# buctcurry/ICKA

Measured on AMD Instinct MI355X. Metric: MNER samples/sec (fwd+bwd) at seq=128, 36 regions, bs=32 per GPU, higher is better.
Workload: dtype bf16; 1 GPU; c2: bert(H768,L12,h12,I3072)+36x2048 regions, seq_len 128, per-GPU batch 32, 1 cross layer(s), gated head, 13 labels, train mode p=0.1, token-CE loss; global_batch=32, seq_len=128, regions=36, parallelism=dp1, launch=hipgraph, precision=bf16, accumulate=1

## Files before the change

### icka_amd/_lib.py

```python
from __future__ import annotations

import ctypes as C
import os
from typing import Optional

_HERE = os.path.dirname(os.path.abspath(__file__))
LIB_PATH = os.path.join(_HERE, "libicka_hip.so")

c_vp, c_i32, c_i64, c_u64, c_f32 = C.c_void_p, C.c_int32, C.c_int64, C.c_uint64, C.c_float

ABI_VERSION = 6
GEMM_NT, GEMM_NN, GEMM_TN, GEMM_TT = 0, 1, 2, 3
ATTN_FP8, ATTN_TILED = 1, 2
LSTM_PER_STEP, LSTM_TICKETS, LSTM_NO_BATCH_SPLIT = 1, 2, 4
EPI_NONE, EPI_GELU, EPI_DGELU, EPI_ADD, EPI_GATE, EPI_TANH, EPI_RELU, EPI_ADD_RELU = 0, 1, 2, 3, 4, 5, 6, 7


class GemmDesc(C.Structure):
    _fields_ = [
        ("op", c_i32), ("M", c_i32), ("N", c_i32), ("K", c_i32), ("K1", c_i32),
        ("A", c_vp), ("lda", c_i64), ("B", c_vp), ("ldb", c_i64),
        ("A2", c_vp), ("lda2", c_i64), ("B2", c_vp), ("ldb2", c_i64),
        ("C", c_vp), ("ldc", c_i64), ("c_is_f32", c_i32),
        ("C2", c_vp), ("ldc2", c_i64),
        ("aux", c_vp), ("ldaux", c_i64),
        ("bias", c_vp), ("bias2", c_vp),
        ("alpha", c_f32), ("beta", c_f32),
        ("epilogue", c_i32),
# ... 228 lines not shown
```

### icka_amd/csrc/attention.hip

```cpp
#include "attn_core.h"

namespace {

__global__ __launch_bounds__(256) void attn_fwd_kernel(const AttnArgs a_) {
    AttnArgs a = a_;
    a.drop = drop_resolve(a.drop);
    __shared__ __attribute__((aligned(16))) char smem[3 * TILE_B];
    char* sQ = smem; char* sK = smem + TILE_B; char* sV = smem + 2 * TILE_B;
    const int tid = threadIdx.x, lane = tid & 63, wave = tid >> 6, g = lane >> 4, i15 = lane & 15;
    const int nqt = (a.Sq + TILE - 1) / TILE;
    const int qt = blockIdx.x % nqt, bh = blockIdx.x / nqt, head = bh % a.h, b = bh / a.h;
    const bf16_t* Qb = a.Q + (int64_t)b * a.Sq * a.ldq + head * HD;
    const bf16_t* Kb = a.K + (int64_t)b * a.Skv * a.ldk + head * HD;
    const bf16_t* Vb = a.V + (int64_t)b * a.Skv * a.ldv + head * HD;
    const float* mb = a.mask + (int64_t)b * a.Skv;

    stage_tile(sQ, Qb, a.ldq, qt * TILE, a.Sq, tid);
    __syncthreads();
    bf16x8 qf[2];
    qf[0] = frag_row(sQ, 16 * wave, 0, lane);
    qf[1] = frag_row(sQ, 16 * wave, 1, lane);
    const int q = qt * TILE + 16 * wave + i15;
    const uint32_t idx_row = ((uint32_t)(b * a.h + head) * (uint32_t)a.Sq + (uint32_t)q) * (uint32_t)a.Skv;

// ... 449 lines not shown
        return;
    }
    if (ICKA_ATTN_ABLATE == 2) {
        for (int i = 0; i < QR * 8 / 256; ++i) {
            const int q = tid + 256 * i, r = q >> 3, c = q & 7;
            if (q0 + r < a.Sq) *reinterpret_cast<u32x4*>(a.Ow + ((int64_t)b * a.Sq + q0 + r) * a.ldo + head * HD + c * 8) =
                *reinterpret_cast<const u32x4*>(sQ + off_t(r, c)) ^ *reinterpret_cast<const u32x4*>(sK + off_t(r % KR, c)) ^
                *reinterpret_cast<const u32x4*>(sV + off_t(r % KR, c));
        }
        return;
    }

    attn_fwd_whole_head<QT, KT, DROP, FP8, KB>(a, sQ, sK, sV, QT * wave, q0, bh, b, head, lane);
}

template <int QT, int KT, bool DROP, bool KB = false, bool VL = false>
__global__ __launch_bounds__(256, (QT * KT >= 36 || QT >= 4 ? 1 : 2)) void attn_bwd_small_kernel(const AttnArgs a_) {
    static_assert(DROP || !KB, "keep bits exist with dropout only");
    static_assert(!(VL && QT * KT >= 36), "packed batches: heads of up to 128 x 128");
    AttnArgs a = a_;
    a.drop = drop_resolve(a.drop);
    constexpr int QR = 64 * QT, KR = 16 * KT, KW = KT / 4;
    constexpr int KV_BYTES = 2 * KR * 128, CH_BYTES = QR * 128;
    constexpr int X_BYTES = KV_BYTES > CH_BYTES ? KV_BYTES : CH_BYTES;
    constexpr int NCAP = (X_BYTES / CH_BYTES) < KW ? (X_BYTES / CH_BYTES) : KW;
    constexpr int NCH = KW % NCAP == 0 ? NCAP : 1;
    constexpr int NG = KW / NCH;
    static_assert(KW % NCH == 0, "chunk groups");
    constexpr bool MASK_LDS = QT * KT >= 36;
    __shared__ __attribute__((aligned(16))) char smem[2 * QR * 128 + X_BYTES + QR * 4 + (MASK_LDS ? KR * 4 : 0)];
    char* sQ = smem; char* sDO = smem + QR * 128; char* sK = sDO + QR * 128; char* sV = sK + KR * 128;
    float* s_lse = reinterpret_cast<float*>(sK + X_BYTES);
    float* s_mask = s_lse + QR;
    const int tid = threadIdx.x, lane = tid & 63, wave = tid >> 6, g = lane >> 4, i15 = lane & 15;
    const int bh = blockIdx.x, head = bh % a.h, b = bh / a.h;
    const float* mb = a.mask + (int64_t)b * a.Skv;
    ATTN_RSTAMP(8);
    ATTN_STAMP(0);
    int qlim = a.Sq, kvlim = a.Skv;
    int64_t q_row0 = (int64_t)b * a.Sq, kv_row0 = (int64_t)b * a.Skv;
    if constexpr (VL) {
        if (bh >= a.B * a.h) {
            const int fb = bh - a.B * a.h;
            vl_zero_filler(a, a.dQ, a.lddq, fb, tid);
            if (a.kv_packed) {
// ... 8 lines not shown
            if (!a.kv_packed) {
                for (int i = tid; i < a.Skv * 8; i += 256) {
                    const int r = i >> 3, c = i & 7;
                    *reinterpret_cast<u32x4*>(a.dK + (kv_row0 + r) * a.lddk + head * HD + c * 8) = u32x4{0u, 0u, 0u, 0u};
                    *reinterpret_cast<u32x4*>(a.dV + (kv_row0 + r) * a.lddv + head * HD + c * 8) = u32x4{0u, 0u, 0u, 0u};
                }
            }
            return;
        }
    }
    stage_rows<QR>(sQ, a.Q + q_row0 * a.ldq + head * HD, a.ldq, qlim, tid);
    stage_rows<QR>(sDO, a.dO + q_row0 * a.lddo + head * HD, a.lddo, qlim, tid);
    stage_rows<KR>(sK, a.K + kv_row0 * a.ldk + head * HD, a.ldk, kvlim, tid);
    stage_rows<KR>(sV, a.V + kv_row0 * a.ldv + head * HD, a.ldv, kvlim, tid);
    if (tid < QR) s_lse[tid] = tid < qlim ? a.lse[(int64_t)bh * a.Sq + tid] : INFINITY;
    if constexpr (MASK_LDS) {
        static_assert(KR <= 256, "one mask element per thread");
        if (tid < KR) s_mask[tid] = tid < a.Skv ? mb[tid] : -INFINITY;
    }
    ATTN_STAMP(1);
    __syncthreads();
    ATTN_STAMP(2);
    if (ICKA_ATTN_ABLATE == 2 && !VL) {
        for (int i = 0; i < QR * 8 / 256; ++i) {
            const int q = tid + 256 * i, r = q >> 3, c = q & 7;
            if (r < a.Sq) *reinterpret_cast<u32x4*>(a.dQ + ((int64_t)b * a.Sq + r) * a.lddq + head * HD + c * 8) =
                *reinterpret_cast<const u32x4*>(sQ + off_t(r, c)) ^ *reinterpret_cast<const u32x4*>(sDO + off_t(r, c));
        }
        for (int i = 0; i < KR * 8 / 256; ++i) {
            const int q = tid + 256 * i, r = q >> 3, c = q & 7;
            if (r < a.Skv) {
                *reinterpret_cast<u32x4*>(a.dK + ((int64_t)b * a.Skv + r) * a.lddk + head * HD + c * 8) =
                    *reinterpret_cast<const u32x4*>(sK + off_t(r, c));
                *reinterpret_cast<u32x4*>(a.dV + ((int64_t)b * a.Skv + r) * a.lddv + head * HD + c * 8) =
                    *reinterpret_cast<const u32x4*>(sV + off_t(r, c));
            }
        }
        return;
    }

    f32x4 mk[MASK_LDS ? 1 : KT];
    if constexpr (!MASK_LDS) {
#pragma unroll
        for (int kt = 0; kt < KT; ++kt)
#pragma unroll
            for (int r = 0; r < 4; ++r) {
                const int key = 16 * kt + 4 * g + r;
                const float mv = mb[key < a.Skv ? key : a.Skv - 1];
                mk[kt][r] = key < a.Skv ? mv : -INFINITY;
            }
    }
    constexpr bool DROP_BITS = MASK_LDS && DROP;
    constexpr int KBW = (KT * 4 + 31) / 32;
    const int wpl = keep_wpl(a.Skv);
    uint32_t dbits[DROP_BITS ? (QT * KT * 4 + 31) / 32 : 1];
    if constexpr (DROP_BITS) {
#pragma unroll
        for (int w = 0; w < (QT * KT * 4 + 31) / 32; ++w) dbits[w] = 0u;
#pragma unroll
        for (int qi = 0; qi < QT; ++qi) {
            const int q = 16 * (QT * wave + qi) + i15;
            const uint32_t idx_row = ((uint32_t)bh * (uint32_t)a.Sq + (uint32_t)q) * (uint32_t)a.Skv;
            const uint32_t hx = (idx_row + 2u * (uint32_t)g) * ICKA_HASH_C0 + a.drop.s0;
            uint32_t kbw[KBW];
            if constexpr (KB) {
// ... 5 lines not shown
            for (int kt = 0; kt < KT; ++kt) {
                const int bit = (qi * KT + kt) * 4;
                uint32_t nib;
                if constexpr (KB) nib = (kbw[(kt * 4) >> 5] >> ((kt * 4) & 31)) & 0xFu;
                else nib = drop_nibble_x<true>(a.drop, hx + (uint32_t)(8 * kt) * ICKA_HASH_C0);
                dbits[bit >> 5] |= nib << (bit & 31);
            }
        }
#pragma unroll
        for (int w = 0; w < (QT * KT * 4 + 31) / 32; ++w) asm volatile("" : "+v"(dbits[w]));
    }
    u32x2 pdp[QT][KT], dsp[QT][KT];
#pragma unroll
    for (int qi = 0; qi < QT; ++qi) {
        const int q = 16 * (QT * wave + qi) + i15;
        if constexpr (VL) {
            if (16 * (QT * wave + qi) >= qlim) {
#pragma unroll
                for (int kt = 0; kt < KT; ++kt) pdp[qi][kt] = dsp[qi][kt] = u32x2{0u, 0u};
                continue;
            }
        }
        const bf16x8 qf0 = frag_row(sQ, 16 * (QT * wave + qi), 0, lane), qf1 = frag_row(sQ, 16 * (QT * wave + qi), 1, lane);
        const bf16x8 do0 = frag_row(sDO, 16 * (QT * wave + qi), 0, lane), do1 = frag_row(sDO, 16 * (QT * wave + qi), 1, lane);
        const float lse_q = s_lse[q];
        const uint32_t idx_row = ((uint32_t)bh * (uint32_t)a.Sq + (uint32_t)q) * (uint32_t)a.Skv;
        const uint32_t hx = (idx_row + 2u * (uint32_t)g) * ICKA_HASH_C0 + a.drop.s0;
        uint32_t kbw[KBW];
        if constexpr (KB && !DROP_BITS) {
            const uint32_t* kp = a.keepbits + (((int64_t)bh * a.Sq + (q < qlim ? q : 0)) * 4 + g) * wpl;
#pragma unroll
            for (int w = 0; w < KBW; ++w) kbw[w] = (w < wpl && q < qlim) ? kp[w] : 0u;
        }
        f32x4 pr[MASK_LDS ? 1 : KT], dpm[KT];
        float dl = 0.f;
#pragma unroll
        for (int kt = 0; kt < KT; ++kt) {
            f32x4 sc = mfma16(frag_row(sK, 16 * kt, 0, lane), qf0, f32x4{0.f, 0.f, 0.f, 0.f});
            sc = mfma16(frag_row(sK, 16 * kt, 1, lane), qf1, sc);
            f32x4 dp = mfma16(frag_row(sV, 16 * kt, 0, lane), do0, f32x4{0.f, 0.f, 0.f, 0.f});
            dp = mfma16(frag_row(sV, 16 * kt, 1, lane), do1, dp);
            f32x4 pd, pvv;
            f32x4 mkv;
            if constexpr (MASK_LDS) mkv = *reinterpret_cast<const f32x4*>(s_mask + 16 * kt + 4 * g);
            else mkv = mk[kt];
            const uint32_t hk = hx + (uint32_t)(8 * kt) * ICKA_HASH_C0;
            if constexpr (MASK_LDS) __builtin_amdgcn_sched_barrier(0);
            float dm4[4];
            if constexpr (!DROP_BITS) {
                if constexpr (KB) {
                    const uint32_t w = kbw[(kt * 4) >> 5], sb = __float_as_uint(a.drop.scale);
#pragma unroll
                    for (int r = 0; r < 4; ++r)
                        dm4[r] = __uint_as_float(sb & (uint32_t)__builtin_amdgcn_sbfe((int)w, ((kt * 4) & 31) + r, 1));
                } else {
                    drop_pair_x<DROP>(a.drop, hk, dm4[0], dm4[1]);
                    drop_pair_x<DROP>(a.drop, hk + ICKA_HASH_C0, dm4[2], dm4[3]);
                }
            }
#pragma unroll
            for (int r = 0; r < 4; ++r) {
                const float pv = __expf(sc[r] * a.scale + mkv[r] - lse_q);
                float dm;
                if constexpr (DROP_BITS) {
                    const int bit = (qi * KT + kt) * 4 + r;
                    dm = ((dbits[bit >> 5] >> (bit & 31)) & 1u) ? a.drop.scale : 0.f;
                } else {
                    dm = dm4[r];
                }
                const float dv = dp[r] * dm;
                pvv[r] = pv;
                dpm[kt][r] = dv;
                pd[r] = pv * dm;
                dl += pv * dv;
            }
            if constexpr (MASK_LDS) {
                pdp[qi][kt] = pack4(pvv[0], pvv[1], pvv[2], pvv[3]);
            } else {
                pr[kt] = pvv;
                pdp[qi][kt] = pack4(pd[0], pd[1], pd[2], pd[3]);
            }
        }
        dl += __shfl_xor(dl, 16, 64);
        dl += __shfl_xor(dl, 32, 64);
        if (g == 0 && q < qlim) a.delta[(int64_t)bh * a.Sq + q] = dl;
#pragma unroll
        for (int kt = 0; kt < KT; ++kt) {
            f32x4 pk;
            if constexpr (MASK_LDS) {
                const bf16x4 pb = as_bf16x4(pdp[qi][kt]);
                pk = f32x4{bf2f(pb[0]), bf2f(pb[1]), bf2f(pb[2]), bf2f(pb[3])};
            } else {
                pk = pr[kt];
            }
            const f32x4 d = pk * (dpm[kt] - dl) * a.scale;
            dsp[qi][kt] = pack4(d[0], d[1], d[2], d[3]);
        }
        f32x4 acc[4];
#pragma unroll
        for (int dt = 0; dt < 4; ++dt) {
            acc[dt] = f32x4{0.f, 0.f, 0.f, 0.f};
#pragma unroll
            for (int ks = 0; ks < KT / 2; ++ks)
                acc[dt] = mfma16(frag_tr(sK, dt, ks, lane),
                                 join8(as_bf16x4(dsp[qi][2 * ks]), as_bf16x4(dsp[qi][2 * ks + 1])), acc[dt]);
        }
        if (q < qlim) {
            bf16_t* row = a.dQ + (q_row0 + q) * a.lddq + head * HD;
#pragma unroll
            for (int dt = 0; dt < 4; ++dt)
                *reinterpret_cast<u32x2*>(row + 16 * dt + 4 * g) = pack4(acc[dt][0], acc[dt][1], acc[dt][2], acc[dt][3]);
        }
    }

    ATTN_STAMP(3);
    char* sX = sK;
    f32x4 acc_k[KW][4], acc_v[KW][4];
#pragma unroll
    for (int kw = 0; kw < KW; ++kw)
#pragma unroll
// ... 61 lines not shown
            if (key < kvlim) {
                bf16_t* krow = a.dK + (kv_row0 + key) * a.lddk + head * HD;
                bf16_t* vrow = a.dV + (kv_row0 + key) * a.lddv + head * HD;
#pragma unroll
                for (int dt = 0; dt < 4; ++dt) {
                    *reinterpret_cast<u32x2*>(krow + 16 * dt + 4 * g) =
                        pack4(acc_k[kw][dt][0], acc_k[kw][dt][1], acc_k[kw][dt][2], acc_k[kw][dt][3]);
                    *reinterpret_cast<u32x2*>(vrow + 16 * dt + 4 * g) =
                        pack4(acc_v[kw][dt][0], acc_v[kw][dt][1], acc_v[kw][dt][2], acc_v[kw][dt][3]);
                }
            }
        }
    ATTN_RSTAMP(9);
}

template <int QT, int KT, bool DROP, bool KB>
static void launch_small2(const AttnArgs& a, int mode, hipStream_t st) {
    if (mode == 1) {
        hipLaunchKernelGGL((attn_bwd_small_kernel<QT, KT, DROP, KB>), dim3(a.B * a.h), dim3(256), 0, st, a);
        return;
    }
    if constexpr (QT > 2) return;
    else if (QT == 2 && (a.B * a.h) % 256 != 0) {
        if (mode == 2) hipLaunchKernelGGL((attn_fwd_small_kernel<1, KT, DROP, true, KB>), dim3(a.B * a.h, 2), dim3(256), 0, st, a);
        else hipLaunchKernelGGL((attn_fwd_small_kernel<1, KT, DROP, false, KB>), dim3(a.B * a.h, 2), dim3(256), 0, st, a);
        return;
    }
    if constexpr (QT <= 2) {
        if (mode == 2) hipLaunchKernelGGL((attn_fwd_small_kernel<QT, KT, DROP, true, KB>), dim3(a.B * a.h), dim3(256), 0, st, a);
        else hipLaunchKernelGGL((attn_fwd_small_kernel<QT, KT, DROP, false, KB>), dim3(a.B * a.h), dim3(256), 0, st, a);
    }
}
template <int QT, int KT>
static void launch_small(const AttnArgs& a, int mode, hipStream_t st) {
    if (a.drop.thr && a.keepbits) launch_small2<QT, KT, true, true>(a, mode, st);
    else if (a.drop.thr) launch_small2<QT, KT, true, false>(a, mode, st);
    else launch_small2<QT, KT, false, false>(a, mode, st);
}
template <int KT>
static void launch_small_fwd_blocks(const AttnArgs& a, hipStream_t st) {
    const dim3 grid(a.B * a.h, (a.Sq + 63) / 64);
    if (a.drop.thr && a.keepbits) hipLaunchKernelGGL((attn_fwd_small_kernel<1, KT, true, false, true>), grid, dim3(256), 0, st, a);
    else if (a.drop.thr) hipLaunchKernelGGL((attn_fwd_small_kernel<1, KT, true, false, false>), grid, dim3(256), 0, st, a);
    else hipLaunchKernelGGL((attn_fwd_small_kernel<1, KT, false, false, false>), grid, dim3(256), 0, st, a);
}
static bool try_small(const AttnArgs& a, int mode, hipStream_t st) {
    if (mode == 0 && a.Skv <= 256 && (a.Sq > 128 || a.Skv > 128)) {
        if (a.Skv > 192) launch_small_fwd_blocks<16>(a, st);
        else if (a.Skv > 128) launch_small_fwd_blocks<12>(a, st);
        else if (a.Skv > 64) launch_small_fwd_blocks<8>(a, st);
        else launch_small_fwd_blocks<4>(a, st);
        return true;
    }
    if (mode == 1 && a.Sq <= 256 && a.Skv <= 256 && (a.Sq > 128 || a.Skv > 128)) {
        if (a.Sq <= 192 && a.Skv <= 192 && a.Skv > 128) launch_small<3, 12>(a, mode, st);
        else if (a.Skv > 128) launch_small<4, 16>(a, mode, st);
        else if (a.Skv > 64) launch_small<4, 8>(a, mode, st);
        else launch_small<4, 4>(a, mode, st);
        return true;
    }
    if (a.Sq > 128 || a.Skv > 128) return false;
    const bool q2 = a.Sq > 64, k8 = a.Skv > 64;
    if (q2 && k8) launch_small<2, 8>(a, mode, st);
    else if (q2) launch_small<2, 4>(a, mode, st);
    else if (k8) launch_small<1, 8>(a, mode, st);
    else launch_small<1, 4>(a, mode, st);
    return true;
}

template <int QT, int KT, bool DROP, bool KB>
static void launch_vl2(const AttnArgs& a, bool bwd, hipStream_t st) {
    const int nb = a.B * a.h + VL_FILL_BLOCKS;
    if (bwd) {
        hipLaunchKernelGGL((attn_bwd_small_kernel<QT, KT, DROP, KB, true>), dim3(nb), dim3(256), 0, st, a);
    } else if (QT == 2 && (a.B * a.h) % 256 != 0) {
        hipLaunchKernelGGL((attn_fwd_small_kernel<1, KT, DROP, false, KB, true>), dim3(nb, 2), dim3(256), 0, st, a);
    } else {
        hipLaunchKernelGGL((attn_fwd_small_kernel<QT, KT, DROP, false, KB, true>), dim3(nb), dim3(256), 0, st, a);
    }
}
template <int QT, int KT>
static void launch_vl(const AttnArgs& a, bool bwd, hipStream_t st) {
    if (a.drop.thr && a.keepbits) launch_vl2<QT, KT, true, true>(a, bwd, st);
    else if (a.drop.thr) launch_vl2<QT, KT, true, false>(a, bwd, st);
    else launch_vl2<QT, KT, false, false>(a, bwd, st);
}
static void try_vl(const AttnArgs& a, bool bwd, hipStream_t st) {
    const bool q2 = a.Sq > 64, k8 = a.Skv > 64;
    if (q2 && k8) launch_vl<2, 8>(a, bwd, st);
    else if (q2) launch_vl<2, 4>(a, bwd, st);
    else if (k8) launch_vl<1, 8>(a, bwd, st);
    else launch_vl<1, 4>(a, bwd, st);
}

inline bool ok16(const void* p, int64_t ld) { return (reinterpret_cast<uintptr_t>(p) & 15) == 0 && ld % 8 == 0; }

#ifdef ICKA_ATTN_STAMP
unsigned long long* g_attn_stamp = nullptr;
#endif

}

#ifdef ICKA_ATTN_STAMP
extern "C" void icka_diag_attn_stamp_buffer(void* p) { g_attn_stamp = (unsigned long long*)p; }
#endif

extern "C" int icka_attn_fwd(const void* Q, int64_t ldq, const void* K, int64_t ldk, const void* V, int64_t ldv,
                             const float* add_mask, void* O, int64_t ldo, float* lse, int32_t B, int32_t heads,
                             int32_t Sq, int32_t Skv, float scale, float p_drop, uint64_t seed, void* stream) {
    if (!Q || !K || !V || !add_mask || !O) return ICKA_E_ARG;
// ... 67 lines not shown
        ICKA_CHECK_LAUNCH();
    }
    return 0;
}
extern "C" int64_t icka_attn_keepbits_words(int32_t B, int32_t heads, int32_t Sq, int32_t Skv) {
    if (B <= 0 || heads <= 0 || Sq <= 0 || Skv <= 0) return 0;
    return (int64_t)B * heads * Sq * 4 * ((Skv + 127) >> 7);
}

extern "C" int icka_attn_bwd(const void* Q, int64_t ldq, const void* K, int64_t ldk, const void* V, int64_t ldv,
                             const float* add_mask, const void* O, int64_t ldo, const void* dO, int64_t lddo,
                             const float* lse, float* delta, void* dQ, int64_t lddq, void* dK, int64_t lddk,
                             void* dV, int64_t lddv, int32_t B, int32_t heads, int32_t Sq, int32_t Skv, float scale,
                             float p_drop, uint64_t seed, const void* keep_bits, int32_t flags, void* stream) {
    if (!Q || !K || !V || !add_mask || !O || !dO || !lse || !delta || !dQ || !dK || !dV) return ICKA_E_ARG;
    if (flags & ~ICKA_ATTN_TILED) return ICKA_E_ARG;
    if (B <= 0 || heads <= 0 || Sq <= 0 || Skv <= 0) return ICKA_E_SHAPE;
    if ((int64_t)B * heads * Sq * Skv >= (1ll << 32)) return ICKA_E_SHAPE;
    if (!ok16(Q, ldq) || !ok16(K, ldk) || !ok16(V, ldv) || !ok16(O, ldo) || !ok16(dO, lddo) || !ok16(dQ, lddq) ||
        !ok16(dK, lddk) || !ok16(dV, lddv))
        return ICKA_E_ALIGN;
    AttnArgs a{};
    a.Q = (const bf16_t*)Q; a.ldq = ldq; a.K = (const bf16_t*)K; a.ldk = ldk; a.V = (const bf16_t*)V; a.ldv = ldv;
    a.mask = add_mask; a.O = (const bf16_t*)O; a.ldo = ldo; a.dO = (const bf16_t*)dO; a.lddo = lddo;
    a.lse = const_cast<float*>(lse); a.delta = delta;
    a.dQ = (bf16_t*)dQ; a.lddq = lddq; a.dK = (bf16_t*)dK; a.lddk = lddk; a.dV = (bf16_t*)dV; a.lddv = lddv;
    a.B = B; a.h = heads; a.Sq = Sq; a.Skv = Skv; a.scale = scale; a.drop = make_drop(p_drop, seed);
    a.keepbits = a.drop.thr ? const_cast<uint32_t*>((const uint32_t*)keep_bits) : nullptr;
    hipStream_t st = (hipStream_t)stream;
#ifdef ICKA_ATTN_STAMP
    a.stamp = g_attn_stamp;
#endif
    if (!(flags & ICKA_ATTN_TILED) && try_small(a, 1, st)) {
        ICKA_CHECK_LAUNCH();
        return 0;
    }
    const dim3 gq(B * heads * ((Sq + TILE - 1) / TILE));
    switch ((Skv + TILE - 1) / TILE) {
        case 1: hipLaunchKernelGGL(attn_bwd_dq_keep_kernel<1>, gq, dim3(256), 0, st, a); break;
        case 2: hipLaunchKernelGGL(attn_bwd_dq_keep_kernel<2>, gq, dim3(256), 0, st, a); break;
        case 3: hipLaunchKernelGGL(attn_bwd_dq_keep_kernel<3>, gq, dim3(256), 0, st, a); break;
        case 4: hipLaunchKernelGGL(attn_bwd_dq_keep_kernel<4>, gq, dim3(256), 0, st, a); break;
        default: hipLaunchKernelGGL(attn_bwd_dq_kernel, gq, dim3(256), 0, st, a); break;
    }
    ICKA_CHECK_LAUNCH();
    hipLaunchKernelGGL(attn_bwd_dkv_kernel, dim3(B * heads * ((Skv + TILE - 1) / TILE)), dim3(256), 0, st, a);
    ICKA_CHECK_LAUNCH();
    return 0;
// ... 17 lines not shown
    a.mask = add_mask; a.Ow = (bf16_t*)O; a.ldo = ldo; a.lse = lse;
    a.B = B; a.h = heads; a.Sq = Sq; a.Skv = Skv; a.scale = scale; a.drop = make_drop(p_drop, seed);
    a.keepbits = a.drop.thr ? (uint32_t*)keep_bits : nullptr;
    a.cu = cu_seqlens; a.kv_packed = kv_packed ? 1 : 0; a.Mrows = Mrows;
    try_vl(a, false, (hipStream_t)stream);
    ICKA_CHECK_LAUNCH();
    return 0;
}
extern "C" int icka_attn_bwd_packed(const void* Q, int64_t ldq, const void* K, int64_t ldk, const void* V, int64_t ldv,
                                    const float* add_mask, const void* dO, int64_t lddo, const float* lse, float* delta,
                                    void* dQ, int64_t lddq, void* dK, int64_t lddk, void* dV, int64_t lddv,
                                    const int32_t* cu_seqlens, int32_t kv_packed, int64_t Mrows, int32_t B, int32_t heads,
                                    int32_t Sq, int32_t Skv, float scale, float p_drop, uint64_t seed, const void* keep_bits,
                                    void* stream) {
    if (!Q || !K || !V || !add_mask || !dO || !lse || !delta || !dQ || !dK || !dV || !cu_seqlens) return ICKA_E_ARG;
    if (const int rc = vl_check(B, heads, Sq, Skv, kv_packed, Mrows)) return rc;
    if (!ok16(Q, ldq) || !ok16(K, ldk) || !ok16(V, ldv) || !ok16(dO, lddo) || !ok16(dQ, lddq) || !ok16(dK, lddk) ||
        !ok16(dV, lddv))
        return ICKA_E_ALIGN;
    AttnArgs a{};
    a.Q = (const bf16_t*)Q; a.ldq = ldq; a.K = (const bf16_t*)K; a.ldk = ldk; a.V = (const bf16_t*)V; a.ldv = ldv;
    a.mask = add_mask; a.dO = (const bf16_t*)dO; a.lddo = lddo;
    a.lse = const_cast<float*>(lse); a.delta = delta;
    a.dQ = (bf16_t*)dQ; a.lddq = lddq; a.dK = (bf16_t*)dK; a.lddk = lddk; a.dV = (bf16_t*)dV; a.lddv = lddv;
    a.B = B; a.h = heads; a.Sq = Sq; a.Skv = Skv; a.scale = scale; a.drop = make_drop(p_drop, seed);
    a.keepbits = a.drop.thr ? const_cast<uint32_t*>((const uint32_t*)keep_bits) : nullptr;
    a.cu = cu_seqlens; a.kv_packed = kv_packed ? 1 : 0; a.Mrows = Mrows;
    try_vl(a, true, (hipStream_t)stream);
    ICKA_CHECK_LAUNCH();
    return 0;
}
```

### icka_amd/kernels.py

```python
from __future__ import annotations

import ctypes as C
import math
from typing import Optional

import torch

from . import _lib
from ._lib import (EPI_ADD, EPI_ADD_RELU, EPI_DGELU, EPI_GATE, EPI_GELU, EPI_NONE, EPI_RELU, EPI_TANH, GEMM_NN, GEMM_NT, GEMM_TN,
                   GemmDesc, check)

BF16 = torch.bfloat16
F32 = torch.float32
F16 = torch.float16


_RAW_STREAM = getattr(torch._C, "_cuda_getCurrentRawStream", None)
_CUR_DEVICE = getattr(torch._C, "_cuda_getDevice", None)


def _stream() -> int:
    if _RAW_STREAM is not None and _CUR_DEVICE is not None:
        return _RAW_STREAM(_CUR_DEVICE())
    return torch.cuda.current_stream().cuda_stream
# ... 550 lines not shown
        if keepbits is not None and (not keepbits.is_cuda or keepbits.element_size() != 4 or not keepbits.is_contiguous()
                                     or keepbits.numel() < lib.icka_attn_keepbits_words(B, heads, Sq, Skv)):
            raise ValueError("keepbits: contiguous 32-bit device buffer of icka_attn_keepbits_words words (attn_keepbits)")
        check(lib.icka_attn_fwd_ex(q.data_ptr(), q.stride(0), k.data_ptr(), k.stride(0), v.data_ptr(), v.stride(0),
                                   add_mask.data_ptr(), out.data_ptr(), _ptr(out16), out.stride(0), _ptr(lse), B, heads,
                                   Sq, Skv, scale, p_drop, seed, (_lib.ATTN_FP8 if fp8 else 0) | (_lib.ATTN_TILED if tiled else 0),
                                   _ptr(keepbits), _stream()), "icka_attn_fwd_ex")
        return out
    fn = lib.icka_attn_fwd_fp8 if fp8 else lib.icka_attn_fwd
    check(fn(q.data_ptr(), q.stride(0), k.data_ptr(), k.stride(0), v.data_ptr(), v.stride(0), add_mask.data_ptr(),
             out.data_ptr(), out.stride(0), _ptr(lse), B, heads, Sq, Skv, scale, p_drop, seed, _stream()),
          "icka_attn_fwd_fp8" if fp8 else "icka_attn_fwd")
    return out


def attn_bwd(q, k, v, add_mask, out, dout, lse, delta, dq, dk, dv, B, heads, Sq, Skv, *, p_drop=0.0, seed=0,
             scale=None, keepbits=None, tiled=False):
    lib = _lib.load()
    for n, t in (("q", q), ("k", k), ("v", v), ("out", out), ("dout", dout), ("dq", dq), ("dk", dk), ("dv", dv)):
        _mat(t, n)
    if scale is None:
        scale = 1.0 / math.sqrt(64.0)
    check(lib.icka_attn_bwd(q.data_ptr(), q.stride(0), k.data_ptr(), k.stride(0), v.data_ptr(), v.stride(0),
                            add_mask.data_ptr(), out.data_ptr(), out.stride(0), dout.data_ptr(), dout.stride(0),
                            lse.data_ptr(), delta.data_ptr(), dq.data_ptr(), dq.stride(0), dk.data_ptr(),
                            dk.stride(0), dv.data_ptr(), dv.stride(0), B, heads, Sq, Skv, scale, p_drop, seed,
                            _ptr(keepbits), _lib.ATTN_TILED if tiled else 0, _stream()), "icka_attn_bwd")


def _i32vec(t: torch.Tensor, n: int, name: str) -> None:
    _dev(t, name)
    if t.dtype != torch.int32 or not t.is_contiguous() or t.numel() < n:
        raise ValueError("%s must be a contiguous int32 device tensor of at least %d elements" % (name, n))


def pack_plan(mask: torch.Tensor, max_tokens: int, plan, err_word: int = 0) -> None:
    _dev(mask, "mask")
    if mask.dtype != torch.int64 or mask.dim() != 2 or not mask.is_contiguous():
        raise ValueError("mask must be a contiguous int64 [B, S] tensor")
    B, S = mask.shape
    _i32vec(plan.lens, B, "lens")
    _i32vec(plan.cu, B + 1, "cu_seqlens")
# ... 71 lines not shown
def attn_bwd_packed(q, k, v, add_mask, dout, lse, delta, dq, dk, dv, cu, kv_packed: bool, B, heads, Sq, Skv, *, p_drop=0.0,
                    seed=0, scale=None, keepbits=None):
    lib = _lib.load()
    for n, t in (("q", q), ("k", k), ("v", v), ("dout", dout), ("dq", dq), ("dk", dk), ("dv", dv)):
        _mat(t, n)
    M = dq.shape[0]
    _packed_checks(B, heads, Sq, Skv, M, kv_packed, add_mask, cu, q=q, dout=dout, dq=dq, k=k, v=v, dk=dk, dv=dv)
    _f32vec(lse, B * heads * Sq, "lse")
    _f32vec(delta, B * heads * Sq, "delta")
    if keepbits is not None and (not keepbits.is_cuda or keepbits.element_size() != 4 or not keepbits.is_contiguous()
                                 or keepbits.numel() < lib.icka_attn_keepbits_words(B, heads, Sq, Skv)):
        raise ValueError("keepbits: contiguous 32-bit device buffer of icka_attn_keepbits_words words (attn_keepbits)")
    check(lib.icka_attn_bwd_packed(q.data_ptr(), q.stride(0), k.data_ptr(), k.stride(0), v.data_ptr(), v.stride(0),
                                   add_mask.data_ptr(), dout.data_ptr(), dout.stride(0), lse.data_ptr(), delta.data_ptr(),
                                   dq.data_ptr(), dq.stride(0), dk.data_ptr(), dk.stride(0), dv.data_ptr(), dv.stride(0),
                                   cu.data_ptr(), int(kv_packed), dq.shape[0], B, heads, Sq, Skv,
                                   (1.0 / 8.0) if scale is None else scale, p_drop, seed, _ptr(keepbits), _stream()),
          "icka_attn_bwd_packed")


def lstm_fwd(gates_x, w_hh, y, c_all, act, hprev, B, S, H, flags=0):
    _dev(gates_x, "gates_x")
    if gates_x.dtype != F32 or gates_x.stride(1) != 1 or tuple(gates_x.shape) != (B * S, 8 * H):
        raise ValueError("gates_x must be f32 [B*S, 8H]")
    for n, t, shp, dt in (("w_hh", w_hh, (8 * H, H), BF16), ("y", y, (B * S, 2 * H), BF16),
                          ("c_all", c_all, (B * S, 2 * H), F32), ("act", act, (B * S, 8 * H), BF16)):
        _dev(t, n)
        if t.dtype != dt or tuple(t.shape) != shp or not t.is_contiguous():
            raise ValueError("%s must be contiguous %s %s" % (n, dt, shp))
    check(_lib.load().icka_lstm_fwd(gates_x.data_ptr(), gates_x.stride(0), w_hh.data_ptr(), y.data_ptr(),
                                    c_all.data_ptr(), act.data_ptr(), _ptr(hprev), B, S, H, int(flags), _stream()), "icka_lstm_fwd")

# ... 595 lines not shown
```

### include/icka_hip.h

```cpp
#ifndef ICKA_HIP_H
#define ICKA_HIP_H

#include <stdint.h>

#ifdef __cplusplus
extern "C" {
#endif

#define ICKA_E_SHAPE (-1)
#define ICKA_E_ALIGN (-2)
#define ICKA_E_ARG (-3)

#define ICKA_ABI_VERSION 6
int icka_abi_version(void);
const char* icka_build_arch(void);

int icka_copy_many(const void* const* src, void* const* dst, const int64_t* bytes, int32_t n, void* stream);

enum { ICKA_GEMM_NT = 0, ICKA_GEMM_NN = 1, ICKA_GEMM_TN = 2 };
enum {
    ICKA_EPI_NONE = 0,
    ICKA_EPI_GELU = 1,
    ICKA_EPI_DGELU = 2,
    ICKA_EPI_ADD = 3,
// ... 96 lines not shown
                          int32_t vocab, int32_t pos_offset, int32_t padding_idx, float p_drop, uint64_t seed,
                          int32_t accumulate, void* stream);

int icka_attn_fwd(const void* Q, int64_t ldq, const void* K, int64_t ldk, const void* V, int64_t ldv,
                  const float* add_mask, void* O, int64_t ldo, float* lse, int32_t B, int32_t heads, int32_t Sq,
                  int32_t Skv, float scale, float p_drop, uint64_t seed, void* stream);
int icka_attn_fwd_fp8(const void* Q, int64_t ldq, const void* K, int64_t ldk, const void* V, int64_t ldv,
                      const float* add_mask, void* O, int64_t ldo, float* lse, int32_t B, int32_t heads, int32_t Sq,
                      int32_t Skv, float scale, float p_drop, uint64_t seed, void* stream);
int icka_attn_fwd_ex(const void* Q, int64_t ldq, const void* K, int64_t ldk, const void* V, int64_t ldv,
                     const float* add_mask, void* O, void* O_f16, int64_t ldo, float* lse, int32_t B, int32_t heads,
                     int32_t Sq, int32_t Skv, float scale, float p_drop, uint64_t seed, int32_t flags, void* keep_bits,
                     void* stream);
#define ICKA_ATTN_FP8 1
#define ICKA_ATTN_TILED 2
int64_t icka_attn_keepbits_words(int32_t B, int32_t heads, int32_t Sq, int32_t Skv);
int icka_attn_bwd(const void* Q, int64_t ldq, const void* K, int64_t ldk, const void* V, int64_t ldv,
                  const float* add_mask, const void* O, int64_t ldo, const void* dO, int64_t lddo, const float* lse,
                  float* delta, void* dQ, int64_t lddq, void* dK, int64_t lddk, void* dV, int64_t lddv, int32_t B,
                  int32_t heads, int32_t Sq, int32_t Skv, float scale, float p_drop, uint64_t seed, const void* keep_bits,
                  int32_t flags, void* stream);

int icka_pack_plan(const int64_t* mask, int32_t B, int32_t S, int32_t max_tokens, int32_t* lens, int32_t* cu_seqlens,
                   int32_t* packed_to_padded, int32_t* padded_to_packed, int32_t* cls_of, int32_t* status, void* err_word,
                   void* stream);
int icka_rows_gather(const void* src, int64_t ld_src, int64_t src_rows, void* dst, int64_t ld_dst, int64_t dst_rows,
                     int32_t row_words, const int32_t* map, int64_t map_stride, uint32_t fill, void* stream);
int icka_attn_fwd_packed(const void* Q, int64_t ldq, const void* K, int64_t ldk, const void* V, int64_t ldv,
                         const float* add_mask, void* O, int64_t ldo, float* lse, const int32_t* cu_seqlens, int32_t kv_packed,
                         int64_t Mrows, int32_t B, int32_t heads, int32_t Sq, int32_t Skv, float scale, float p_drop,
// ... 206 lines not shown
```

Baseline: 7314 samples/s.

## Skip masked key tiles and zero-gradient query tiles in small attention backward

Adds a SKIP variant of the small attention backward kernel. It skips a whole 16-query tile when its dO fragment is all zeros, and skips the dP MFMAs and softmax work for key tiles whose masked scores all fall far below the logsumexp. Candidate key tiles are found up front with a wave ballot on the mask. The variant is on by default through an env var and a flag, and is excluded for the QT=1,KT=8 config. The checks cost extra branches, LDS mask staging and a duplicated code path (larger code, register pressure), and the skip treats exp of very negative values as exactly zero.

Result: no change. 7250 samples/s (-0.9%).

```diff
diff --git a/icka_amd/_lib.py b/icka_amd/_lib.py
--- a/icka_amd/_lib.py
+++ b/icka_amd/_lib.py
@@ -12,6 +12,7 @@
 ABI_VERSION = 6
 GEMM_NT, GEMM_NN, GEMM_TN, GEMM_TT = 0, 1, 2, 3
 ATTN_FP8, ATTN_TILED = 1, 2
+ATTN_NOSKIP = 4
 LSTM_PER_STEP, LSTM_TICKETS, LSTM_NO_BATCH_SPLIT = 1, 2, 4
 EPI_NONE, EPI_GELU, EPI_DGELU, EPI_ADD, EPI_GATE, EPI_TANH, EPI_RELU, EPI_ADD_RELU = 0, 1, 2, 3, 4, 5, 6, 7
 
diff --git a/icka_amd/csrc/attention.hip b/icka_amd/csrc/attention.hip
--- a/icka_amd/csrc/attention.hip
+++ b/icka_amd/csrc/attention.hip
@@ -487,7 +487,8 @@
     attn_fwd_whole_head<QT, KT, DROP, FP8, KB>(a, sQ, sK, sV, QT * wave, q0, bh, b, head, lane);
 }
 
-template <int QT, int KT, bool DROP, bool KB = false, bool VL = false>
+constexpr float SKIP_MASK_T = -100.f, SKIP_X_ZERO = -128.f;
+template <int QT, int KT, bool DROP, bool KB = false, bool VL = false, bool SKIP = false>
 __global__ __launch_bounds__(256, (QT * KT >= 36 || QT >= 4 ? 1 : 2)) void attn_bwd_small_kernel(const AttnArgs a_) {
     static_assert(DROP || !KB, "keep bits exist with dropout only");
     static_assert(!(VL && QT * KT >= 36), "packed batches: heads of up to 128 x 128");
@@ -501,7 +502,8 @@
     constexpr int NG = KW / NCH;
     static_assert(KW % NCH == 0, "chunk groups");
     constexpr bool MASK_LDS = QT * KT >= 36;
-    __shared__ __attribute__((aligned(16))) char smem[2 * QR * 128 + X_BYTES + QR * 4 + (MASK_LDS ? KR * 4 : 0)];
+    constexpr bool MASK_SMEM = MASK_LDS || SKIP;
+    __shared__ __attribute__((aligned(16))) char smem[2 * QR * 128 + X_BYTES + QR * 4 + (MASK_SMEM ? KR * 4 : 0)];
     char* sQ = smem; char* sDO = smem + QR * 128; char* sK = sDO + QR * 128; char* sV = sK + KR * 128;
     float* s_lse = reinterpret_cast<float*>(sK + X_BYTES);
     float* s_mask = s_lse + QR;
@@ -540,7 +542,7 @@
     stage_rows<KR>(sK, a.K + kv_row0 * a.ldk + head * HD, a.ldk, kvlim, tid);
     stage_rows<KR>(sV, a.V + kv_row0 * a.ldv + head * HD, a.ldv, kvlim, tid);
     if (tid < QR) s_lse[tid] = tid < qlim ? a.lse[(int64_t)bh * a.Sq + tid] : INFINITY;
-    if constexpr (MASK_LDS) {
+    if constexpr (MASK_SMEM) {
         static_assert(KR <= 256, "one mask element per thread");
         if (tid < KR) s_mask[tid] = tid < a.Skv ? mb[tid] : -INFINITY;
     }
@@ -565,8 +567,8 @@
         return;
     }
 
-    f32x4 mk[MASK_LDS ? 1 : KT];
-    if constexpr (!MASK_LDS) {
+    f32x4 mk[MASK_SMEM ? 1 : KT];
+    if constexpr (!MASK_SMEM) {
 #pragma unroll
         for (int kt = 0; kt < KT; ++kt)
 #pragma unroll
@@ -575,6 +577,14 @@
                 const float mv = mb[key < a.Skv ? key : a.Skv - 1];
                 mk[kt][r] = key < a.Skv ? mv : -INFINITY;
             }
+    }
+    uint32_t cand = 0u;
+    if constexpr (SKIP) {
+#pragma unroll
+        for (int kt = 0; kt < KT; ++kt) {
+            cand |= (__ballot(s_mask[16 * kt + i15] < SKIP_MASK_T) != 0ull ? 1u : 0u) << kt;
+        }
+        cand = __builtin_amdgcn_readfirstlane(cand);
     }
     constexpr bool DROP_BITS = MASK_LDS && DROP;
     constexpr int KBW = (KT * 4 + 31) / 32;
@@ -610,7 +620,7 @@
 #pragma unroll
     for (int qi = 0; qi < QT; ++qi) {
         const int q = 16 * (QT * wave + qi) + i15;
-        if constexpr (VL) {
+        if constexpr (VL && !SKIP) {
             if (16 * (QT * wave + qi) >= qlim) {
 #pragma unroll
                 for (int kt = 0; kt < KT; ++kt) pdp[qi][kt] = dsp[qi][kt] = u32x2{0u, 0u};
@@ -619,87 +629,125 @@
         }
         const bf16x8 qf0 = frag_row(sQ, 16 * (QT * wave + qi), 0, lane), qf1 = frag_row(sQ, 16 * (QT * wave + qi), 1, lane);
         const bf16x8 do0 = frag_row(sDO, 16 * (QT * wave + qi), 0, lane), do1 = frag_row(sDO, 16 * (QT * wave + qi), 1, lane);
-        const float lse_q = s_lse[q];
-        const uint32_t idx_row = ((uint32_t)bh * (uint32_t)a.Sq + (uint32_t)q) * (uint32_t)a.Skv;
-        const uint32_t hx = (idx_row + 2u * (uint32_t)g) * ICKA_HASH_C0 + a.drop.s0;
-        uint32_t kbw[KBW];
-        if constexpr (KB && !DROP_BITS) {
-            const uint32_t* kp = a.keepbits + (((int64_t)bh * a.Sq + (q < qlim ? q : 0)) * 4 + g) * wpl;
-#pragma unroll
-            for (int w = 0; w < KBW; ++w) kbw[w] = (w < wpl && q < qlim) ? kp[w] : 0u;
-        }
-        f32x4 pr[MASK_LDS ? 1 : KT], dpm[KT];
+        bool qskip = false;
+        if constexpr (SKIP) {
+            const u32x4 d0 = __builtin_bit_cast(u32x4, do0), d1 = __builtin_bit_cast(u32x4, do1);
+            const uint32_t nz = (d0[0] | d0[1] | d0[2] | d0[3] | d1[0] | d1[1] | d1[2] | d1[3]) & 0x7fff7fffu;
+            qskip = __all(nz == 0u);
+            if constexpr (VL) qskip = qskip || 16 * (QT * wave + qi) >= qlim;
+        }
         float dl = 0.f;
-#pragma unroll
-        for (int kt = 0; kt < KT; ++kt) {
-            f32x4 sc = mfma16(frag_row(sK, 16 * kt, 0, lane), qf0, f32x4{0.f, 0.f, 0.f, 0.f});
-            sc = mfma16(frag_row(sK, 16 * kt, 1, lane), qf1, sc);
-            f32x4 dp = mfma16(frag_row(sV, 16 * kt, 0, lane), do0, f32x4{0.f, 0.f, 0.f, 0.f});
-            dp = mfma16(frag_row(sV, 16 * kt, 1, lane), do1, dp);
-            f32x4 pd, pvv;
-            f32x4 mkv;
-            if constexpr (MASK_LDS) mkv = *reinterpret_cast<const f32x4*>(s_mask + 16 * kt + 4 * g);
-            else mkv = mk[kt];
-            const uint32_t hk = hx + (uint32_t)(8 * kt) * ICKA_HASH_C0;
-            if constexpr (MASK_LDS) __builtin_amdgcn_sched_barrier(0);
-            float dm4[4];
-            if constexpr (!DROP_BITS) {
-                if constexpr (KB) {
-                    const uint32_t w = kbw[(kt * 4) >> 5], sb = __float_as_uint(a.drop.scale);
-#pragma unroll
-                    for (int r = 0; r < 4; ++r)
-                        dm4[r] = __uint_as_float(sb & (uint32_t)__builtin_amdgcn_sbfe((int)w, ((kt * 4) & 31) + r, 1));
+        f32x4 acc[4];
+        if (qskip) {
+#pragma unroll
+            for (int dt = 0; dt < 4; ++dt) acc[dt] = f32x4{0.f, 0.f, 0.f, 0.f};
+#pragma unroll
+            for (int kt = 0; kt < KT; ++kt) pdp[qi][kt] = dsp[qi][kt] = u32x2{0u, 0u};
+        } else {
+            const float lse_q = s_lse[q];
+            const uint32_t idx_row = ((uint32_t)bh * (uint32_t)a.Sq + (uint32_t)q) * (uint32_t)a.Skv;
+            const uint32_t hx = (idx_row + 2u * (uint32_t)g) * ICKA_HASH_C0 + a.drop.s0;
+            uint32_t kbw[KBW];
+            if constexpr (KB && !DROP_BITS) {
+                const uint32_t* kp = a.keepbits + (((int64_t)bh * a.Sq + (q < qlim ? q : 0)) * 4 + g) * wpl;
+#pragma unroll
+                for (int w = 0; w < KBW; ++w) kbw[w] = (w < wpl && q < qlim) ? kp[w] : 0u;
+            }
+            f32x4 pr[MASK_LDS ? 1 : KT], dpm[KT];
+#pragma unroll
+            for (int copy = 0; copy < (SKIP ? 2 : 1); ++copy) {
+                const bool CHECK = SKIP && copy == 0;
+                if (SKIP && CHECK != (cand != 0u)) continue;
+#pragma unroll
+                for (int kt = 0; kt < KT; ++kt) {
+                    f32x4 sc = mfma16(frag_row(sK, 16 * kt, 0, lane), qf0, f32x4{0.f, 0.f, 0.f, 0.f});
+                    sc = mfma16(frag_row(sK, 16 * kt, 1, lane), qf1, sc);
+                    f32x4 mkv;
+                    if constexpr (MASK_SMEM) mkv = *reinterpret_cast<const f32x4*>(s_mask + 16 * kt + 4 * g);
+                    else mkv = mk[kt];
+                    if (CHECK) {
+                        if ((cand >> kt) & 1u) {
+                            bool below = true;
+#pragma unroll
+                            for (int r = 0; r < 4; ++r)
+                                below = below && (__builtin_fmaf(sc[r], a.scale, mkv[r]) - lse_q < SKIP_X_ZERO);
+                            if (__all(below)) {
+                                pdp[qi][kt] = u32x2{0u, 0u};
+                                dpm[kt] = f32x4{0.f, 0.f, 0.f, 0.f};
+                                if constexpr (!MASK_LDS) pr[kt] = f32x4{0.f, 0.f, 0.f, 0.f};
+                                continue;
+                            }
+                        }
+                    }
+                    f32x4 dp = mfma16(frag_row(sV, 16 * kt, 0, lane), do0, f32x4{0.f, 0.f, 0.f, 0.f});
+                    dp = mfma16(frag_row(sV, 16 * kt, 1, lane), do1, dp);
+                    f32x4 pd, pvv;
+                    const uint32_t hk = hx + (uint32_t)(8 * kt) * ICKA_HASH_C0;
+                    if constexpr (MASK_LDS) __builtin_amdgcn_sched_barrier(0);
+                    float dm4[4];
+                    if constexpr (!DROP_BITS) {
+                        if constexpr (KB) {
+                            const uint32_t w = kbw[(kt * 4) >> 5], sb = __float_as_uint(a.drop.scale);
+#pragma unroll
+                            for (int r = 0; r < 4; ++r)
+                                dm4[r] = __uint_as_float(sb & (uint32_t)__builtin_amdgcn_sbfe((int)w, ((kt * 4) & 31) + r, 1));
+                        } else {
+                            drop_pair_x<DROP>(a.drop, hk, dm4[0], dm4[1]);
+                            drop_pair_x<DROP>(a.drop, hk + ICKA_HASH_C0, dm4[2], dm4[3]);
+                        }
+                    }
+#pragma unroll
+                    for (int r = 0; r < 4; ++r) {
+                            const float pv = __expf(__builtin_fmaf(sc[r], a.scale, mkv[r]) - lse_q);
+                        float dm;
+                        if constexpr (DROP_BITS) {
+                            const int bit = (qi * KT + kt) * 4 + r;
+                            dm = ((dbits[bit >> 5] >> (bit & 31)) & 1u) ? a.drop.scale : 0.f;
+                        } else {
+                            dm = dm4[r];
+                        }
+                        const float dv = dp[r] * dm;
+                        pvv[r] = pv;
+                        dpm[kt][r] = dv;
+                        pd[r] = pv * dm;
+                        dl = __builtin_fmaf(pv, dv, dl);
+                    }
+                    if constexpr (MASK_LDS) {
+                        pdp[qi][kt] = pack4(pvv[0], pvv[1], pvv[2], pvv[3]);
+                    } else {
+                        pr[kt] = pvv;
+                        pdp[qi][kt] = pack4(pd[0], pd[1], pd[2], pd[3]);
+                    }
+                }
+            }
+            dl += __shfl_xor(dl, 16, 64);
+            dl += __shfl_xor(dl, 32, 64);
+            if constexpr (!SKIP) {
+                if (g == 0 && q < qlim) a.delta[(int64_t)bh * a.Sq + q] = dl;
+            }
+#pragma unroll
+            for (int kt = 0; kt < KT; ++kt) {
+                f32x4 pk;
+                if constexpr (MASK_LDS) {
+                    const bf16x4 pb = as_bf16x4(pdp[qi][kt]);
+                    pk = f32x4{bf2f(pb[0]), bf2f(pb[1]), bf2f(pb[2]), bf2f(pb[3])};
                 } else {
-                    drop_pair_x<DROP>(a.drop, hk, dm4[0], dm4[1]);
-                    drop_pair_x<DROP>(a.drop, hk + ICKA_HASH_C0, dm4[2], dm4[3]);
+                    pk = pr[kt];
                 }
-            }
-#pragma unroll
-            for (int r = 0; r < 4; ++r) {
-                const float pv = __expf(sc[r] * a.scale + mkv[r] - lse_q);
-                float dm;
-                if constexpr (DROP_BITS) {
-                    const int bit = (qi * KT + kt) * 4 + r;
-                    dm = ((dbits[bit >> 5] >> (bit & 31)) & 1u) ? a.drop.scale : 0.f;
-                } else {
-                    dm = dm4[r];
-                }
-                const float dv = dp[r] * dm;
-                pvv[r] = pv;
-                dpm[kt][r] = dv;
-                pd[r] = pv * dm;
-                dl += pv * dv;
-            }
-            if constexpr (MASK_LDS) {
-                pdp[qi][kt] = pack4(pvv[0], pvv[1], pvv[2], pvv[3]);
-            } else {
-                pr[kt] = pvv;
-                pdp[qi][kt] = pack4(pd[0], pd[1], pd[2], pd[3]);
-            }
-        }
-        dl += __shfl_xor(dl, 16, 64);
-        dl += __shfl_xor(dl, 32, 64);
-        if (g == 0 && q < qlim) a.delta[(int64_t)bh * a.Sq + q] = dl;
-#pragma unroll
-        for (int kt = 0; kt < KT; ++kt) {
-            f32x4 pk;
-            if constexpr (MASK_LDS) {
-                const bf16x4 pb = as_bf16x4(pdp[qi][kt]);
-                pk = f32x4{bf2f(pb[0]), bf2f(pb[1]), bf2f(pb[2]), bf2f(pb[3])};
-            } else {
-                pk = pr[kt];
-            }
-            const f32x4 d = pk * (dpm[kt] - dl) * a.scale;
-            dsp[qi][kt] = pack4(d[0], d[1], d[2], d[3]);
-        }
-        f32x4 acc[4];
-#pragma unroll
-        for (int dt = 0; dt < 4; ++dt) {
-            acc[dt] = f32x4{0.f, 0.f, 0.f, 0.f};
-#pragma unroll
-            for (int ks = 0; ks < KT / 2; ++ks)
-                acc[dt] = mfma16(frag_tr(sK, dt, ks, lane),
-                                 join8(as_bf16x4(dsp[qi][2 * ks]), as_bf16x4(dsp[qi][2 * ks + 1])), acc[dt]);
+                const f32x4 d = pk * (dpm[kt] - dl) * a.scale;
+                dsp[qi][kt] = pack4(d[0], d[1], d[2], d[3]);
+            }
+#pragma unroll
+            for (int dt = 0; dt < 4; ++dt) {
+                acc[dt] = f32x4{0.f, 0.f, 0.f, 0.f};
+#pragma unroll
+                for (int ks = 0; ks < KT / 2; ++ks)
+                    acc[dt] = mfma16(frag_tr(sK, dt, ks, lane),
+                                     join8(as_bf16x4(dsp[qi][2 * ks]), as_bf16x4(dsp[qi][2 * ks + 1])), acc[dt]);
+            }
+        }
+        if constexpr (SKIP) {
+            if (g == 0 && q < qlim) a.delta[(int64_t)bh * a.Sq + q] = dl;
         }
         if (q < qlim) {
             bf16_t* row = a.dQ + (q_row0 + q) * a.lddq + head * HD;
@@ -791,9 +839,17 @@
     ATTN_RSTAMP(9);
 }
 
+template <int QT, int KT>
+constexpr bool SKIP_OK = !(QT == 1 && KT == 8);
 template <int QT, int KT, bool DROP, bool KB>
-static void launch_small2(const AttnArgs& a, int mode, hipStream_t st) {
+static void launch_small2(const AttnArgs& a, int mode, hipStream_t st, bool skip) {
     if (mode == 1) {
+        if constexpr (SKIP_OK<QT, KT>) {
+            if (skip) {
+                hipLaunchKernelGGL((attn_bwd_small_kernel<QT, KT, DROP, KB, false, true>), dim3(a.B * a.h), dim3(256), 0, st, a);
+                return;
+            }
+        }
         hipLaunchKernelGGL((attn_bwd_small_kernel<QT, KT, DROP, KB>), dim3(a.B * a.h), dim3(256), 0, st, a);
         return;
     }
@@ -809,10 +865,10 @@
     }
 }
 template <int QT, int KT>
-static void launch_small(const AttnArgs& a, int mode, hipStream_t st) {
-    if (a.drop.thr && a.keepbits) launch_small2<QT, KT, true, true>(a, mode, st);
-    else if (a.drop.thr) launch_small2<QT, KT, true, false>(a, mode, st);
-    else launch_small2<QT, KT, false, false>(a, mode, st);
+static void launch_small(const AttnArgs& a, int mode, hipStream_t st, bool skip) {
+    if (a.drop.thr && a.keepbits) launch_small2<QT, KT, true, true>(a, mode, st, skip);
+    else if (a.drop.thr) launch_small2<QT, KT, true, false>(a, mode, st, skip);
+    else launch_small2<QT, KT, false, false>(a, mode, st, skip);
 }
 template <int KT>
 static void launch_small_fwd_blocks(const AttnArgs& a, hipStream_t st) {
@@ -821,7 +877,7 @@
     else if (a.drop.thr) hipLaunchKernelGGL((attn_fwd_small_kernel<1, KT, true, false, false>), grid, dim3(256), 0, st, a);
     else hipLaunchKernelGGL((attn_fwd_small_kernel<1, KT, false, false, false>), grid, dim3(256), 0, st, a);
 }
-static bool try_small(const AttnArgs& a, int mode, hipStream_t st) {
+static bool try_small(const AttnArgs& a, int mode, hipStream_t st, bool skip = false) {
     if (mode == 0 && a.Skv <= 256 && (a.Sq > 128 || a.Skv > 128)) {
         if (a.Skv > 192) launch_small_fwd_blocks<16>(a, st);
         else if (a.Skv > 128) launch_small_fwd_blocks<12>(a, st);
@@ -830,25 +886,31 @@
         return true;
     }
     if (mode == 1 && a.Sq <= 256 && a.Skv <= 256 && (a.Sq > 128 || a.Skv > 128)) {
-        if (a.Sq <= 192 && a.Skv <= 192 && a.Skv > 128) launch_small<3, 12>(a, mode, st);
-        else if (a.Skv > 128) launch_small<4, 16>(a, mode, st);
-        else if (a.Skv > 64) launch_small<4, 8>(a, mode, st);
-        else launch_small<4, 4>(a, mode, st);
+        if (a.Sq <= 192 && a.Skv <= 192 && a.Skv > 128) launch_small<3, 12>(a, mode, st, skip);
+        else if (a.Skv > 128) launch_small<4, 16>(a, mode, st, skip);
+        else if (a.Skv > 64) launch_small<4, 8>(a, mode, st, skip);
+        else launch_small<4, 4>(a, mode, st, skip);
         return true;
     }
     if (a.Sq > 128 || a.Skv > 128) return false;
     const bool q2 = a.Sq > 64, k8 = a.Skv > 64;
-    if (q2 && k8) launch_small<2, 8>(a, mode, st);
-    else if (q2) launch_small<2, 4>(a, mode, st);
-    else if (k8) launch_small<1, 8>(a, mode, st);
-    else launch_small<1, 4>(a, mode, st);
+    if (q2 && k8) launch_small<2, 8>(a, mode, st, skip);
+    else if (q2) launch_small<2, 4>(a, mode, st, skip);
+    else if (k8) launch_small<1, 8>(a, mode, st, skip);
+    else launch_small<1, 4>(a, mode, st, skip);
     return true;
 }
 
 template <int QT, int KT, bool DROP, bool KB>
-static void launch_vl2(const AttnArgs& a, bool bwd, hipStream_t st) {
+static void launch_vl2(const AttnArgs& a, bool bwd, hipStream_t st, bool skip) {
     const int nb = a.B * a.h + VL_FILL_BLOCKS;
     if (bwd) {
+        if constexpr (SKIP_OK<QT, KT>) {
+            if (skip) {
+                hipLaunchKernelGGL((attn_bwd_small_kernel<QT, KT, DROP, KB, true, true>), dim3(nb), dim3(256), 0, st, a);
+                return;
+            }
+        }
         hipLaunchKernelGGL((attn_bwd_small_kernel<QT, KT, DROP, KB, true>), dim3(nb), dim3(256), 0, st, a);
     } else if (QT == 2 && (a.B * a.h) % 256 != 0) {
         hipLaunchKernelGGL((attn_fwd_small_kernel<1, KT, DROP, false, KB, true>), dim3(nb, 2), dim3(256), 0, st, a);
@@ -857,20 +919,28 @@
     }
 }
 template <int QT, int KT>
-static void launch_vl(const AttnArgs& a, bool bwd, hipStream_t st) {
-    if (a.drop.thr && a.keepbits) launch_vl2<QT, KT, true, true>(a, bwd, st);
-    else if (a.drop.thr) launch_vl2<QT, KT, true, false>(a, bwd, st);
-    else launch_vl2<QT, KT, false, false>(a, bwd, st);
-}
-static void try_vl(const AttnArgs& a, bool bwd, hipStream_t st) {
+static void launch_vl(const AttnArgs& a, bool bwd, hipStream_t st, bool skip) {
+    if (a.drop.thr && a.keepbits) launch_vl2<QT, KT, true, true>(a, bwd, st, skip);
+    else if (a.drop.thr) launch_vl2<QT, KT, true, false>(a, bwd, st, skip);
+    else launch_vl2<QT, KT, false, false>(a, bwd, st, skip);
+}
+static void try_vl(const AttnArgs& a, bool bwd, hipStream_t st, bool skip = false) {
     const bool q2 = a.Sq > 64, k8 = a.Skv > 64;
-    if (q2 && k8) launch_vl<2, 8>(a, bwd, st);
-    else if (q2) launch_vl<2, 4>(a, bwd, st);
-    else if (k8) launch_vl<1, 8>(a, bwd, st);
-    else launch_vl<1, 4>(a, bwd, st);
+    if (q2 && k8) launch_vl<2, 8>(a, bwd, st, skip);
+    else if (q2) launch_vl<2, 4>(a, bwd, st, skip);
+    else if (k8) launch_vl<1, 8>(a, bwd, st, skip);
+    else launch_vl<1, 4>(a, bwd, st, skip);
 }
 
 inline bool ok16(const void* p, int64_t ld) { return (reinterpret_cast<uintptr_t>(p) & 15) == 0 && ld % 8 == 0; }
+
+inline bool attn_skip_default() {
+    static const bool on = [] {
+        const char* e = getenv("ICKA_ATTN_SKIP");
+        return !(e && e[0] == '0');
+    }();
+    return on;
+}
 
 #ifdef ICKA_ATTN_STAMP
 unsigned long long* g_attn_stamp = nullptr;
@@ -968,7 +1038,7 @@
                              void* dV, int64_t lddv, int32_t B, int32_t heads, int32_t Sq, int32_t Skv, float scale,
                              float p_drop, uint64_t seed, const void* keep_bits, int32_t flags, void* stream) {
     if (!Q || !K || !V || !add_mask || !O || !dO || !lse || !delta || !dQ || !dK || !dV) return ICKA_E_ARG;
-    if (flags & ~ICKA_ATTN_TILED) return ICKA_E_ARG;
+    if (flags & ~(ICKA_ATTN_TILED | ICKA_ATTN_NOSKIP)) return ICKA_E_ARG;
     if (B <= 0 || heads <= 0 || Sq <= 0 || Skv <= 0) return ICKA_E_SHAPE;
     if ((int64_t)B * heads * Sq * Skv >= (1ll << 32)) return ICKA_E_SHAPE;
     if (!ok16(Q, ldq) || !ok16(K, ldk) || !ok16(V, ldv) || !ok16(O, ldo) || !ok16(dO, lddo) || !ok16(dQ, lddq) ||
@@ -985,7 +1055,7 @@
 #ifdef ICKA_ATTN_STAMP
     a.stamp = g_attn_stamp;
 #endif
-    if (!(flags & ICKA_ATTN_TILED) && try_small(a, 1, st)) {
+    if (!(flags & ICKA_ATTN_TILED) && try_small(a, 1, st, !(flags & ICKA_ATTN_NOSKIP) && attn_skip_default())) {
         ICKA_CHECK_LAUNCH();
         return 0;
     }
@@ -1033,6 +1103,8 @@
                                     int32_t Sq, int32_t Skv, float scale, float p_drop, uint64_t seed, const void* keep_bits,
                                     void* stream) {
     if (!Q || !K || !V || !add_mask || !dO || !lse || !delta || !dQ || !dK || !dV || !cu_seqlens) return ICKA_E_ARG;
+    const bool noskip = (kv_packed & ICKA_ATTN_NOSKIP) != 0;
+    kv_packed &= ~ICKA_ATTN_NOSKIP;
     if (const int rc = vl_check(B, heads, Sq, Skv, kv_packed, Mrows)) return rc;
     if (!ok16(Q, ldq) || !ok16(K, ldk) || !ok16(V, ldv) || !ok16(dO, lddo) || !ok16(dQ, lddq) || !ok16(dK, lddk) ||
         !ok16(dV, lddv))
@@ -1045,7 +1117,7 @@
     a.B = B; a.h = heads; a.Sq = Sq; a.Skv = Skv; a.scale = scale; a.drop = make_drop(p_drop, seed);
     a.keepbits = a.drop.thr ? const_cast<uint32_t*>((const uint32_t*)keep_bits) : nullptr;
     a.cu = cu_seqlens; a.kv_packed = kv_packed ? 1 : 0; a.Mrows = Mrows;
-    try_vl(a, true, (hipStream_t)stream);
+    try_vl(a, true, (hipStream_t)stream, !noskip && attn_skip_default());
     ICKA_CHECK_LAUNCH();
     return 0;
 }
diff --git a/icka_amd/kernels.py b/icka_amd/kernels.py
--- a/icka_amd/kernels.py
+++ b/icka_amd/kernels.py
@@ -588,6 +588,15 @@
     return out
 
 
+_ATTN_SKIP = True
+
+
+def attn_set_skip(on: bool) -> bool:
+    global _ATTN_SKIP
+    prev, _ATTN_SKIP = _ATTN_SKIP, bool(on)
+    return prev
+
+
 def attn_bwd(q, k, v, add_mask, out, dout, lse, delta, dq, dk, dv, B, heads, Sq, Skv, *, p_drop=0.0, seed=0,
              scale=None, keepbits=None, tiled=False):
     lib = _lib.load()
@@ -599,7 +608,8 @@
                             add_mask.data_ptr(), out.data_ptr(), out.stride(0), dout.data_ptr(), dout.stride(0),
                             lse.data_ptr(), delta.data_ptr(), dq.data_ptr(), dq.stride(0), dk.data_ptr(),
                             dk.stride(0), dv.data_ptr(), dv.stride(0), B, heads, Sq, Skv, scale, p_drop, seed,
-                            _ptr(keepbits), _lib.ATTN_TILED if tiled else 0, _stream()), "icka_attn_bwd")
+                            _ptr(keepbits), (_lib.ATTN_TILED if tiled else 0) | (0 if _ATTN_SKIP else _lib.ATTN_NOSKIP),
+                            _stream()), "icka_attn_bwd")
 
 
 def _i32vec(t: torch.Tensor, n: int, name: str) -> None:
@@ -701,8 +711,8 @@
     check(lib.icka_attn_bwd_packed(q.data_ptr(), q.stride(0), k.data_ptr(), k.stride(0), v.data_ptr(), v.stride(0),
                                    add_mask.data_ptr(), dout.data_ptr(), dout.stride(0), lse.data_ptr(), delta.data_ptr(),
                                    dq.data_ptr(), dq.stride(0), dk.data_ptr(), dk.stride(0), dv.data_ptr(), dv.stride(0),
-                                   cu.data_ptr(), int(kv_packed), dq.shape[0], B, heads, Sq, Skv,
-                                   (1.0 / 8.0) if scale is None else scale, p_drop, seed, _ptr(keepbits), _stream()),
+                                   cu.data_ptr(), int(bool(kv_packed)) | (0 if _ATTN_SKIP else _lib.ATTN_NOSKIP), dq.shape[0],
+                                   B, heads, Sq, Skv, (1.0 / 8.0) if scale is None else scale, p_drop, seed, _ptr(keepbits), _stream()),
           "icka_attn_bwd_packed")
 
 
diff --git a/include/icka_hip.h b/include/icka_hip.h
--- a/include/icka_hip.h
+++ b/include/icka_hip.h
@@ -134,6 +134,7 @@
                      void* stream);
 #define ICKA_ATTN_FP8 1
 #define ICKA_ATTN_TILED 2
+#define ICKA_ATTN_NOSKIP 4
 int64_t icka_attn_keepbits_words(int32_t B, int32_t heads, int32_t Sq, int32_t Skv);
 int icka_attn_bwd(const void* Q, int64_t ldq, const void* K, int64_t ldk, const void* V, int64_t ldv,
                   const float* add_mask, const void* O, int64_t ldo, const void* dO, int64_t lddo, const float* lse,
```
